# MahdiGhafoorian/NLML_HPE

Measured on AMD Instinct MI355X. Metric: faces_per_sec, higher is better.
Workload: dtype f16x2s

## Files before the change

nlml_hpe_amd/csrc/encoder_heads_f16x2_tailws_dev.h:

```cpp
#pragma once
#include <hip/hip_runtime.h>

#include "../../include/nlml_hpe.h"
#include "abi_internal.h"
#include "encoder_heads_f16x2_dev.h"
#include "layout.h"

#if defined(__HIP_DEVICE_COMPILE__) && !defined(__gfx950__)
#error "global_load_lds_dwordx4: gfx950"
#endif

namespace nlml {
namespace hx {

typedef unsigned u4 __attribute__((ext_vector_type(4)));
#define TW_PRIO(p) __builtin_amdgcn_s_setprio(p)
typedef __attribute__((address_space(3))) const char LdsC;
typedef __attribute__((address_space(3))) char LdsW;

struct TwArgs {
  const void* blob;
  const u4* h3;
  float* out;
  float* latent;
  int64_t B, nfb;
};

constexpr int TW_SLOT = 65536;
constexpr int tw_bias_n16(int s) { return kStages[s].jobs * kStages[s].nb * 8; }
constexpr int tw_bias_off(int s) {
  int o = 0;
  for (int t = ST_E3; t < s; ++t) o += tw_bias_n16(t) * 16;
  return o;
}
constexpr uint32_t tw_b_off(int s, uint32_t k16_e0) {
  int c = (int)(sizeof(Header) / 16), m = 0;
  for (int t = 0; t < s; ++t) {
    c += kStages[t].jobs * ((t == ST_E0 ? 0 : kStages[t].k8 * kStages[t].nb * 64 * PIECES) + kStages[t].nb * 8);
    m += kStages[t].jobs * (t == ST_E0 ? kStages[t].nb * 64 * PIECES : 0);
  }
  return c + m * k16_e0 + kStages[s].jobs * ((s == ST_E0 ? 0 : kStages[s].k8 * kStages[s].nb * 64 * PIECES) + (s == ST_E0 ? kStages[s].nb * 64 * PIECES : 0) * k16_e0);
}
constexpr bool tw_b_off_is_layouts() {
  for (int s = 0; s < NUM_STAGES; ++s)
    if (tw_b_off(s, 0u) != layout_b_off(kLayoutHX, s, 0u) || tw_b_off(s, 88u) != layout_b_off(kLayoutHX, s, 88u)) return false;
  return true;
}
static_assert(tw_b_off_is_layouts(), "the written-out bias offsets are layout.h's");
constexpr int TW_O_BIAS = 2 * TW_SLOT;
constexpr int TW_O_LAT = TW_O_BIAS + ((tw_bias_off(NUM_STAGES) + 511) / 512) * 512;
constexpr int TW_LAT_WAVE = 3 * 2 * 256;
constexpr int TW_LDS = TW_O_LAT + 8 * TW_LAT_WAVE;
static_assert(TW_LDS <= 163840, "LDS map");

constexpr int TW_HEAD_UNITS = 9, TW_UNITS = 4 + 3 * TW_HEAD_UNITS;
constexpr uint32_t tw_job_w16(int s) { return layout_job_w16(kLayoutHX, s, 0u); }
__device__ __forceinline__ void tw_unit(const HdrRegs& H, int idx, uint32_t& off, uint32_t& n16) {
  constexpr uint32_t J3 = tw_job_w16(ST_E3), J4 = tw_job_w16(ST_E4), J5 = tw_job_w16(ST_E5);
  constexpr uint32_t K0 = tw_job_w16(ST_H0), K1 = tw_job_w16(ST_H1), K2 = tw_job_w16(ST_H2), K3 = tw_job_w16(ST_H3), K4 = tw_job_w16(ST_H4);
  static_assert(2 * J3 * 16 == TW_SLOT && 2 * J4 * 16 <= TW_SLOT && J5 * 16 <= TW_SLOT && 4 * K0 * 16 <= TW_SLOT && K1 * 16 <= TW_SLOT &&
                    2 * K2 * 16 == TW_SLOT && 2 * K3 * 16 <= TW_SLOT && K4 * 16 <= TW_SLOT,
                "a unit fits a buffer");
  if (idx < 2) { n16 = 2 * J3; off = H.w_off(ST_E3) + idx * 2 * J3; }
  else if (idx == 2) { n16 = 2 * J4; off = H.w_off(ST_E4); }
  else if (idx == 3) { n16 = J5; off = H.w_off(ST_E5); }
  else {
    const int k = idx - 4, g = k / TW_HEAD_UNITS, r = k - TW_HEAD_UNITS * g;
    if (r == 0) { n16 = 4 * K0; off = H.w_off(ST_H0) + 4 * g * K0; }
    else if (r <= 4) { n16 = K1; off = H.w_off(ST_H1) + (4 * g + (r - 1)) * K1; }
    else if (r <= 6) { n16 = 2 * K2; off = H.w_off(ST_H2) + (4 * g + 2 * (r - 5)) * K2; }
    else if (r == 7) { n16 = 2 * K3; off = H.w_off(ST_H3) + 2 * g * K3; }
    else { n16 = K4; off = H.w_off(ST_H4) + g * K4; }
  }
}

template <int K16, int NCH = 2>
__device__ __forceinline__ void tw_job2(f32x16 (&acc)[2], LdsC* w0, LdsC* w1, int wstep, LdsC* b0, LdsC* b1, const h8 (&in)[K16][2]) {
  typedef const __attribute__((address_space(3))) h8 LdsH8;
#pragma unroll
  for (int c = 0; c < NCH; ++c)
#pragma unroll
    for (int q = 0; q < 4; ++q) {
      const f32x4 v = *reinterpret_cast<const __attribute__((address_space(3))) f32x4*>((c ? b1 : b0) + q * 16);
      acc[c][4 * q + 0] = v[0];
      acc[c][4 * q + 1] = v[1];
      acc[c][4 * q + 2] = v[2];
      acc[c][4 * q + 3] = v[3];
    }
  TW_PRIO(2);
#pragma unroll
  for (int ks = 0; ks < K16; ++ks) {
    h8 wf[NCH][2];
#pragma unroll
    for (int c = 0; c < NCH; ++c)
#pragma unroll
      for (int p = 0; p < 2; ++p) wf[c][p] = *reinterpret_cast<LdsH8*>((c ? w1 : w0) + ks * wstep + p * 1024);
#pragma unroll
    for (int t = 0; t < 3; ++t)
#pragma unroll
      for (int c = 0; c < NCH; ++c)
        acc[c] = __builtin_amdgcn_mfma_f32_32x32x16_f16(wf[c][t == 0 ? 1 : 0], in[ks][t == 1 ? 1 : 0], acc[c], 0, 0, 0);
  }
  TW_PRIO(0);
}

template <int K16>
__device__ __forceinline__ void tw_job2p(f32x16 (&acc)[2], LdsC* w0, LdsC* w1, int wstep, LdsC* b0, LdsC* b1, const h8 (&in)[K16][2]) {
  typedef const __attribute__((address_space(3))) h8 LdsH8;
#pragma unroll
  for (int c = 0; c < 2; ++c)
#pragma unroll
    for (int q = 0; q < 4; ++q) {
      const f32x4 v = *reinterpret_cast<const __attribute__((address_space(3))) f32x4*>((c ? b1 : b0) + q * 16);
      acc[c][4 * q + 0] = v[0];
      acc[c][4 * q + 1] = v[1];
      acc[c][4 * q + 2] = v[2];
      acc[c][4 * q + 3] = v[3];
    }
  h8 wf[2][2][2];
#pragma unroll
  for (int c = 0; c < 2; ++c)
#pragma unroll
    for (int p = 0; p < 2; ++p) wf[0][c][p] = *reinterpret_cast<LdsH8*>((c ? w1 : w0) + p * 1024);
  TW_PRIO(2);
  __builtin_amdgcn_sched_barrier(0);
#pragma unroll
  for (int ks = 0; ks < K16; ++ks) {
#pragma unroll
    for (int m = 0; m < 6; ++m) {
      const int t = m >> 1, c = m & 1;
      acc[c] = __builtin_amdgcn_mfma_f32_32x32x16_f16(wf[ks & 1][c][t == 0 ? 1 : 0], in[ks][t == 1 ? 1 : 0], acc[c], 0, 0, 0);
      __builtin_amdgcn_sched_barrier(0);
      if (m < 4 && ks + 1 < K16)
        wf[(ks + 1) & 1][m & 1][m < 2 ? 1 : 0] = *reinterpret_cast<LdsH8*>(((m & 1) ? w1 : w0) + (ks + 1) * wstep + (m < 2 ? 1024 : 0));
      __builtin_amdgcn_sched_barrier(0);
    }
  }
  TW_PRIO(0);
}

__device__ __forceinline__ void tail_ws_body(const TwArgs& a, int64_t block0, char* const lds) {
  const int tid = threadIdx.x, lane = tid & 63, f = lane & 31, h = lane >> 5;
  const int wv = __builtin_amdgcn_readfirstlane(tid >> 6);
  const HdrRegs H = load_hdr(reinterpret_cast<const Header*>(a.blob));
  const h8* const blob8 = reinterpret_cast<const h8*>(a.blob);
  const f32x4* const blob4 = reinterpret_cast<const f32x4*>(a.blob);

  int64_t fbg = block0 + wv;
  const bool wave_live = fbg < a.nfb;
  fbg = wave_live ? fbg : a.nfb - 1;
  const int64_t row = fbg * 32 + f;
  const bool row_live = wave_live && row < a.B;

  LdsW* const ring = (LdsW*)(lds);
  auto issue = [&](int idx, int slot_off) {
    if (idx >= TW_UNITS) return;
    uint32_t off, n16;
    tw_unit(H, idx, off, n16);
    const int npieces = (int)(n16 >> 6);
#pragma unroll
    for (int i = 0; i < TW_SLOT / 8192; ++i) {
      const int pc = wv + 8 * i;
      if (pc < npieces)
        __builtin_amdgcn_global_load_lds((const __attribute__((address_space(1))) void*)(blob8 + off + pc * 64 + lane),
                                         (__attribute__((address_space(3))) void*)(ring + slot_off + pc * 1024), 16, 0, 0);
    }
  };
#ifdef TW_STAMPS
  int tw_u = 0;
#define TWS(i)                                                                                                                \
  do {                                                                                                                        \
    if (a.latent && lane == 0)                                                                                                \
      reinterpret_cast<unsigned long long*>(a.latent)[((size_t)blockIdx.x * 8 + wv) * 96 + (i)] = __builtin_amdgcn_s_memtime(); \
  } while (0)
#define TW_STAMP_MID() TWS(2 + 2 * tw_u)
#define TW_STAMP_END() do { TWS(3 + 2 * tw_u); ++tw_u; } while (0)
#else
#define TWS(i) do { } while (0)
#define TW_STAMP_MID() do { } while (0)
#define TW_STAMP_END() do { } while (0)
#endif
  TWS(0);
  issue(0, 0);

  {
    f32x4* const bl = reinterpret_cast<f32x4*>(lds + TW_O_BIAS);
#pragma unroll
    for (int s = ST_E3; s < NUM_STAGES; ++s) {
      const f32x4* src = blob4 + tw_b_off(s, H.k8_e0);
      for (int i = tid; i < tw_bias_n16(s); i += 512) bl[tw_bias_off(s) / 16 + i] = src[i];
    }
  }
  h8 x3[TrunkFrags::STEPS][2];
  {
    const u4* src = a.h3 + TrunkFrags::unit(fbg, 0, 0, 0) + lane;
#pragma unroll
    for (int ks = 0; ks < TrunkFrags::STEPS; ++ks)
#pragma unroll
      for (int p = 0; p < 2; ++p) x3[ks][p] = __builtin_bit_cast(h8, src[TrunkFrags::frag(0, ks, p)]);
  }
  asm volatile("s_waitcnt vmcnt(0)" ::: "memory");
  __syncthreads();
  TWS(1);

  int cur = 0;
  LdsC* const bias0 = (LdsC*)(lds + TW_O_BIAS) + 64 * h;
  LdsC* const wl0 = (LdsC*)(lds) + lane * 16;
  LdsW* const latw = (LdsW*)(lds + TW_O_LAT) + wv * TW_LAT_WAVE + f * 8;
#ifdef TW_NO_SKEW
  const bool late = false;
#else
  const bool late = wv >= 4;
#endif
#define TW_BEGIN(idx) issue((idx) + 1, cur ^ TW_SLOT); LdsC* const wl = wl0 + cur
#define TW_MID()                                      \
  TW_STAMP_MID();                                     \
  asm volatile("s_waitcnt vmcnt(0)" ::: "memory");    \
  if (late) __syncthreads()
#define TW_END()                                      \
  asm volatile("s_waitcnt vmcnt(0)" ::: "memory");    \
  if (!late) __syncthreads();                         \
  TW_STAMP_END();                                     \
  cur ^= TW_SLOT

  f32x16 acc[2];
  auto emit = [&](auto act, const f32x16& ac, float inv, h8 (&d0)[2], h8 (&d1)[2]) {
    h8 fr[2][2];
    frags_from_acc<decltype(act)::value>(ac, inv, fr);
    d0[0] = fr[0][0]; d0[1] = fr[0][1]; d1[0] = fr[1][0]; d1[1] = fr[1][1];
  };
  constexpr std::integral_constant<int, ACT_RELU> RELU{};
  constexpr std::integral_constant<int, ACT_TANH> TANH{};
  const float inv3 = H.inv_scale[ST_E3], inv4 = H.inv_scale[ST_E4], inv5 = H.inv_scale[ST_E5];
  constexpr int JB3 = (int)(tw_job_w16(ST_E3) * 16), JB4 = (int)(tw_job_w16(ST_E4) * 16);

  h8 x4[8][2];
#pragma unroll
  for (int u = 0; u < 2; ++u) {
    TW_BEGIN(u);
    LdsC* const b = bias0 + tw_bias_off(ST_E3) + (2 * u) * 128;
    tw_job2p<16>(acc, wl, wl + JB3, 2048, b, b + 128, x3);
    TW_MID();
    emit(RELU, acc[0], inv3, x4[4 * u], x4[4 * u + 1]);
    emit(RELU, acc[1], inv3, x4[4 * u + 2], x4[4 * u + 3]);
    TW_END();
  }
  h8 x5[4][2];
  {
    TW_BEGIN(2);
    LdsC* const b = bias0 + tw_bias_off(ST_E4);
    tw_job2<8>(acc, wl, wl + JB4, 2048, b, b + 128, x4);
    TW_MID();
    emit(TANH, acc[0], inv4, x5[0], x5[1]);
    emit(TANH, acc[1], inv4, x5[2], x5[3]);
    TW_END();
  }
  {
    TW_BEGIN(3);
    LdsC* const b = bias0 + tw_bias_off(ST_E5);
    tw_job2<4>(acc, wl, wl + 2048, 4096, b, b + 128, x5);
    TW_MID();
#ifndef TW_STAMPS
    if (a.latent && row_live) {
#pragma unroll
      for (int nb = 0; nb < 2; ++nb)
#pragma unroll
        for (int q = 0; q < 16; ++q) {
          const int rowi = 32 * nb + (q & 3) + 8 * (q >> 2) + 4 * h, g = rowi >> 4, cc = rowi & 15;
          if (g < 3 && cc < 3) a.latent[row * NLML_LATENT + 3 * g + cc] = acc[nb][q] * inv5;
        }
    }
#endif
#pragma unroll
    for (int nb = 0; nb < 2; ++nb) {
      h8 fr[2][2];
      frags_from_acc<ACT_NONE>(acc[nb], inv5, fr);
#pragma unroll
      for (int p = 0; p < 2; ++p)
#pragma unroll
        for (int pc = 0; pc < 2; ++pc)
          if (2 * nb + p < 3 && h == 0) {
            const u4 t = __builtin_bit_cast(u4, fr[p][pc]);
            typedef unsigned u2 __attribute__((ext_vector_type(2)));
            *reinterpret_cast<__attribute__((address_space(3))) u2*>(latw + ((2 * nb + p) * 2 + pc) * 256) = u2{t[0], t[1]};
          }
    }
    TW_END();
  }
#pragma unroll 1
  for (int g = 0; g < 3; ++g) {
    const int u0 = 4 + TW_HEAD_UNITS * g;
    const float i0 = H.inv_scale[ST_H0], i1 = H.inv_scale[ST_H1], i2 = H.inv_scale[ST_H2], i3 = H.inv_scale[ST_H3];
    h8 xa[8][2];
    {
      TW_BEGIN(u0);
      h8 xin[1][2];
#pragma unroll
      for (int pc = 0; pc < 2; ++pc) {
        typedef unsigned u2 __attribute__((ext_vector_type(2)));
        const u2 t = *reinterpret_cast<const __attribute__((address_space(3))) u2*>((LdsC*)latw + (g * 2 + pc) * 256);
        xin[0][pc] = __builtin_bit_cast(h8, u4{h == 0 ? t[0] : 0u, h == 0 ? t[1] : 0u, 0u, 0u});
      }
      LdsC* const b = bias0 + tw_bias_off(ST_H0) + (4 * g) * 128;
      constexpr int JB = (int)(tw_job_w16(ST_H0) * 16);
#pragma unroll
      for (int jj = 0; jj < 2; ++jj) {
        tw_job2<1>(acc, wl + (2 * jj) * JB, wl + (2 * jj + 1) * JB, 2048, b + (2 * jj) * 128, b + (2 * jj + 1) * 128, xin);
        if (jj == 1) { TW_MID(); }
        emit(RELU, acc[0], i0, xa[4 * jj], xa[4 * jj + 1]);
        emit(RELU, acc[1], i0, xa[4 * jj + 2], xa[4 * jj + 3]);
      }
      TW_END();
    }
    h8 xb[16][2];
#pragma unroll
    for (int j = 0; j < 4; ++j) {
      TW_BEGIN(u0 + 1 + j);
      LdsC* const b = bias0 + tw_bias_off(ST_H1) + (4 * g + j) * 256;
      tw_job2p<8>(acc, wl, wl + 2048, 4096, b, b + 128, xa);
      TW_MID();
      emit(RELU, acc[0], i1, xb[4 * j], xb[4 * j + 1]);
      emit(RELU, acc[1], i1, xb[4 * j + 2], xb[4 * j + 3]);
      TW_END();
    }
    h8 xc[8][2];
#pragma unroll
    for (int u = 0; u < 2; ++u) {
      TW_BEGIN(u0 + 5 + u);
      constexpr int JB = (int)(tw_job_w16(ST_H2) * 16);
      LdsC* const b = bias0 + tw_bias_off(ST_H2) + (4 * g + 2 * u) * 128;
      tw_job2p<16>(acc, wl, wl + JB, 2048, b, b + 128, xb);
      TW_MID();
      emit(RELU, acc[0], i2, xc[4 * u], xc[4 * u + 1]);
      emit(RELU, acc[1], i2, xc[4 * u + 2], xc[4 * u + 3]);
      TW_END();
    }
    h8 xd[4][2];
    {
      TW_BEGIN(u0 + 7);
      LdsC* const b = bias0 + tw_bias_off(ST_H3) + (2 * g) * 128;
      tw_job2p<8>(acc, wl, wl + (int)(tw_job_w16(ST_H3) * 16), 2048, b, b + 128, xc);
      TW_MID();
      emit(RELU, acc[0], i3, xd[0], xd[1]);
      emit(RELU, acc[1], i3, xd[2], xd[3]);
      TW_END();
    }
    {
      TW_BEGIN(u0 + 8);
      LdsC* const b = bias0 + tw_bias_off(ST_H4) + g * 128;
      tw_job2<4, 1>(acc, wl, wl, 2048, b, b, xd);
      TW_MID();
      if (h == 0 && row_live) a.out[row * 3 + g] = acc[0][0] * H.inv_scale[ST_H4];
      TW_END();
    }
  }
#undef TW_BEGIN
#undef TW_MID
#undef TW_END
}

}
}
```

Before: 81.14 million.

## Merge small tail weight units into shared LDS buffers to cut barriers

Packs small consecutive weight units (E4+E5+H0, and H3+H4+next H0) into single double-buffered LDS slots, so the tail goes from 31 units to 24. This removes several waitcnt/__syncthreads seams and prefetch handoffs between tiny jobs. A constexpr checker verifies that the units cover the tail weights in order and fit a slot. The cost is larger per-unit loads with less prefetch lead for the following job, plus more complex control flow.

```diff
diff --git a/nlml_hpe_amd/csrc/encoder_heads_f16x2_tailws_dev.h b/nlml_hpe_amd/csrc/encoder_heads_f16x2_tailws_dev.h
--- a/nlml_hpe_amd/csrc/encoder_heads_f16x2_tailws_dev.h
+++ b/nlml_hpe_amd/csrc/encoder_heads_f16x2_tailws_dev.h
@@ -53,26 +53,70 @@
 constexpr int TW_LDS = TW_O_LAT + 8 * TW_LAT_WAVE;
 static_assert(TW_LDS <= 163840, "LDS map");
 
-constexpr int TW_HEAD_UNITS = 9, TW_UNITS = 4 + 3 * TW_HEAD_UNITS;
+struct TwSeg { int stage, job0, jobs; };
+struct TwUnit { TwSeg seg[3]; };
+#ifdef TW_NO_MERGE
+constexpr int TW_ENC_UNITS = 4, TW_HEAD_UNITS = 9;
+#else
+constexpr int TW_ENC_UNITS = 3, TW_HEAD_UNITS = 7;
+#endif
+constexpr int TW_KINDS = TW_ENC_UNITS + TW_HEAD_UNITS, TW_UNITS = TW_ENC_UNITS + 3 * TW_HEAD_UNITS;
+#ifdef TW_NO_MERGE
+constexpr int TW_K_E4 = 2, TW_K_E5 = 3, TW_K_H0 = 4, TW_K_H1 = 5, TW_K_H2 = 9, TW_K_H3 = 11, TW_K_H4 = 12;
+#else
+constexpr int TW_K_E4 = 2, TW_K_E5 = 2, TW_K_H1 = 3, TW_K_H2 = 7, TW_K_H3 = 9, TW_K_H4 = 9;
+#endif
+constexpr TwUnit tw_unit(int k, int g) {
+  if (k < 2) return {{{ST_E3, 2 * k, 2}, {}, {}}};
+#ifdef TW_NO_MERGE
+  if (k == TW_K_E4) return {{{ST_E4, 0, 2}, {}, {}}};
+  if (k == TW_K_E5) return {{{ST_E5, 0, 1}, {}, {}}};
+  if (k == TW_K_H0) return {{{ST_H0, 4 * g, 4}, {}, {}}};
+  if (k < TW_K_H2) return {{{ST_H1, 4 * g + (k - TW_K_H1), 1}, {}, {}}};
+  if (k < TW_K_H3) return {{{ST_H2, 4 * g + 2 * (k - TW_K_H2), 2}, {}, {}}};
+  if (k == TW_K_H3) return {{{ST_H3, 2 * g, 2}, {}, {}}};
+  return {{{ST_H4, g, 1}, {}, {}}};
+#else
+  if (k == TW_K_E4) return {{{ST_E4, 0, 2}, {ST_E5, 0, 1}, {ST_H0, 0, 4}}};
+  if (k < TW_K_H2) return {{{ST_H1, 4 * g + (k - TW_K_H1), 1}, {}, {}}};
+  if (k < TW_K_H3) return {{{ST_H2, 4 * g + 2 * (k - TW_K_H2), 2}, {}, {}}};
+  return {{{ST_H3, 2 * g, 2}, {ST_H4, g, 1}, {ST_H0, 4 * (g + 1), g < 2 ? 4 : 0}}};
+#endif
+}
 constexpr uint32_t tw_job_w16(int s) { return layout_job_w16(kLayoutHX, s, 0u); }
-__device__ __forceinline__ void tw_unit(const HdrRegs& H, int idx, uint32_t& off, uint32_t& n16) {
-  constexpr uint32_t J3 = tw_job_w16(ST_E3), J4 = tw_job_w16(ST_E4), J5 = tw_job_w16(ST_E5);
-  constexpr uint32_t K0 = tw_job_w16(ST_H0), K1 = tw_job_w16(ST_H1), K2 = tw_job_w16(ST_H2), K3 = tw_job_w16(ST_H3), K4 = tw_job_w16(ST_H4);
-  static_assert(2 * J3 * 16 == TW_SLOT && 2 * J4 * 16 <= TW_SLOT && J5 * 16 <= TW_SLOT && 4 * K0 * 16 <= TW_SLOT && K1 * 16 <= TW_SLOT &&
-                    2 * K2 * 16 == TW_SLOT && 2 * K3 * 16 <= TW_SLOT && K4 * 16 <= TW_SLOT,
-                "a unit fits a buffer");
-  if (idx < 2) { n16 = 2 * J3; off = H.w_off(ST_E3) + idx * 2 * J3; }
-  else if (idx == 2) { n16 = 2 * J4; off = H.w_off(ST_E4); }
-  else if (idx == 3) { n16 = J5; off = H.w_off(ST_E5); }
-  else {
-    const int k = idx - 4, g = k / TW_HEAD_UNITS, r = k - TW_HEAD_UNITS * g;
-    if (r == 0) { n16 = 4 * K0; off = H.w_off(ST_H0) + 4 * g * K0; }
-    else if (r <= 4) { n16 = K1; off = H.w_off(ST_H1) + (4 * g + (r - 1)) * K1; }
-    else if (r <= 6) { n16 = 2 * K2; off = H.w_off(ST_H2) + (4 * g + 2 * (r - 5)) * K2; }
-    else if (r == 7) { n16 = 2 * K3; off = H.w_off(ST_H3) + 2 * g * K3; }
-    else { n16 = K4; off = H.w_off(ST_H4) + g * K4; }
-  }
-}
+constexpr int tw_seg_pieces(const TwSeg& s) { return s.jobs * (int)(tw_job_w16(s.stage) >> 6); }
+constexpr bool tw_units_are_the_tail() {
+  int next[NUM_STAGES] = {};
+  for (int idx = 0; idx < TW_UNITS; ++idx) {
+    const int k = idx < TW_ENC_UNITS ? idx : TW_ENC_UNITS + (idx - TW_ENC_UNITS) % TW_HEAD_UNITS;
+    const int g = idx < TW_ENC_UNITS ? 0 : (idx - TW_ENC_UNITS) / TW_HEAD_UNITS;
+    const TwUnit U = tw_unit(k, g);
+    int pieces = 0;
+    for (int j = 0; j < 3; ++j) {
+      const TwSeg s = U.seg[j];
+      if (s.jobs == 0) continue;
+      if (s.stage < ST_E3 || s.stage >= NUM_STAGES || s.job0 != next[s.stage] || tw_seg_pieces(s) % 8 != 0) return false;
+      if ((tw_job_w16(s.stage) & 63u) != 0) return false;
+      if (s.stage > ST_E3) {
+        const int p = s.stage - 1;
+        const int need = s.stage <= ST_H0 ? kStages[p].jobs : ((s.job0 + s.jobs - 1) / (kStages[s.stage].jobs / 3) + 1) * (kStages[p].jobs / 3);
+        if (next[p] < need) return false;
+      }
+      next[s.stage] += s.jobs;
+      pieces += tw_seg_pieces(s);
+    }
+    if (pieces == 0 || pieces * 1024 > TW_SLOT) return false;
+  }
+  for (int s = ST_E3; s < NUM_STAGES; ++s)
+    if (next[s] != kStages[s].jobs) return false;
+  return true;
+}
+static_assert(tw_units_are_the_tail(), "the units cover the tail's weights exactly once, in the order of use, each within a buffer");
+#ifndef TW_NO_MERGE
+static_assert(TW_UNITS == 24 && (2 * tw_job_w16(ST_E4) + tw_job_w16(ST_E5) + 4 * tw_job_w16(ST_H0)) * 16 == 56 * 1024 &&
+                  (2 * tw_job_w16(ST_H3) + tw_job_w16(ST_H4) + 4 * tw_job_w16(ST_H0)) * 16 == 48 * 1024,
+              "E4 + E5 + H0 is 56 KB, H3 + H4 + H0 is 48 KB");
+#endif
 
 template <int K16, int NCH = 2>
 __device__ __forceinline__ void tw_job2(f32x16 (&acc)[2], LdsC* w0, LdsC* w1, int wstep, LdsC* b0, LdsC* b1, const h8 (&in)[K16][2]) {
@@ -153,18 +197,30 @@
   const bool row_live = wave_live && row < a.B;
 
   LdsW* const ring = (LdsW*)(lds);
-  auto issue = [&](int idx, int slot_off) {
-    if (idx >= TW_UNITS) return;
-    uint32_t off, n16;
-    tw_unit(H, idx, off, n16);
-    const int npieces = (int)(n16 >> 6);
-#pragma unroll
-    for (int i = 0; i < TW_SLOT / 8192; ++i) {
-      const int pc = wv + 8 * i;
-      if (pc < npieces)
-        __builtin_amdgcn_global_load_lds((const __attribute__((address_space(1))) void*)(blob8 + off + pc * 64 + lane),
-                                         (__attribute__((address_space(3))) void*)(ring + slot_off + pc * 1024), 16, 0, 0);
-    }
+  auto issue = [&](int k, int g, int slot_off) {
+    const TwUnit U = tw_unit(k, g);
+    int first = 0;
+    unsigned lane16 = lane * 16;
+    asm volatile("" : "+v"(lane16));
+#pragma unroll
+    for (int j = 0; j < 3; ++j) {
+      const int np = tw_seg_pieces(U.seg[j]);
+      const uint32_t off = H.w_off(U.seg[j].stage) + U.seg[j].job0 * tw_job_w16(U.seg[j].stage);
+#pragma unroll
+      for (int i = 0; i < TW_SLOT / 8192; ++i) {
+        const int pc = wv + 8 * i;
+        if (8 * i >= first && 8 * i < first + np) {
+          const char* const piece = reinterpret_cast<const char*>(a.blob) + (size_t)(off + (pc - first) * 64) * 16;
+          __builtin_amdgcn_global_load_lds((const __attribute__((address_space(1))) void*)(piece + lane16),
+                                           (__attribute__((address_space(3))) void*)(ring + slot_off + pc * 1024), 16, 0, 0);
+        }
+      }
+      first += np;
+    }
+  };
+  auto issue_next = [&](int k, int g, int slot_off) {
+    if (k + 1 < TW_KINDS) issue(k + 1, g, slot_off);
+    else if (g < 2) issue(TW_ENC_UNITS, g + 1, slot_off);
   };
 #ifdef TW_STAMPS
   int tw_u = 0;
@@ -181,7 +237,7 @@
 #define TW_STAMP_END() do { } while (0)
 #endif
   TWS(0);
-  issue(0, 0);
+  issue(0, 0, 0);
 
   {
     f32x4* const bl = reinterpret_cast<f32x4*>(lds + TW_O_BIAS);
@@ -212,7 +268,8 @@
 #else
   const bool late = wv >= 4;
 #endif
-#define TW_BEGIN(idx) issue((idx) + 1, cur ^ TW_SLOT); LdsC* const wl = wl0 + cur
+  LdsC* wl;
+#define TW_BEGIN(k, g) issue_next(k, g, cur ^ TW_SLOT); wl = wl0 + cur
 #define TW_MID()                                      \
   TW_STAMP_MID();                                     \
   asm volatile("s_waitcnt vmcnt(0)" ::: "memory");    \
@@ -222,6 +279,13 @@
   if (!late) __syncthreads();                         \
   TW_STAMP_END();                                     \
   cur ^= TW_SLOT
+#ifdef TW_NO_MERGE
+#define TW_SEAM_MID() TW_MID()
+#define TW_SEAM_END(k, g, bytes) TW_END(); TW_BEGIN(k, g)
+#else
+#define TW_SEAM_MID() do { } while (0)
+#define TW_SEAM_END(k, g, bytes) wl += (bytes)
+#endif
 
   f32x16 acc[2];
   auto emit = [&](auto act, const f32x16& ac, float inv, h8 (&d0)[2], h8 (&d1)[2]) {
@@ -232,12 +296,32 @@
   constexpr std::integral_constant<int, ACT_RELU> RELU{};
   constexpr std::integral_constant<int, ACT_TANH> TANH{};
   const float inv3 = H.inv_scale[ST_E3], inv4 = H.inv_scale[ST_E4], inv5 = H.inv_scale[ST_E5];
-  constexpr int JB3 = (int)(tw_job_w16(ST_E3) * 16), JB4 = (int)(tw_job_w16(ST_E4) * 16);
+  constexpr int JB3 = (int)(tw_job_w16(ST_E3) * 16), JB4 = (int)(tw_job_w16(ST_E4) * 16), JB5 = (int)(tw_job_w16(ST_E5) * 16);
+  constexpr int JBH0 = (int)(tw_job_w16(ST_H0) * 16), JBH3 = (int)(tw_job_w16(ST_H3) * 16), JBH4 = (int)(tw_job_w16(ST_H4) * 16);
+
+  auto h0_front = [&](int gg, LdsC* w, h8 (&xa)[8][2]) {
+    h8 xin[1][2];
+#pragma unroll
+    for (int pc = 0; pc < 2; ++pc) {
+      typedef unsigned u2 __attribute__((ext_vector_type(2)));
+      const u2 t = *reinterpret_cast<const __attribute__((address_space(3))) u2*>((LdsC*)latw + (gg * 2 + pc) * 256);
+      xin[0][pc] = __builtin_bit_cast(h8, u4{h == 0 ? t[0] : 0u, h == 0 ? t[1] : 0u, 0u, 0u});
+    }
+    LdsC* const b = bias0 + tw_bias_off(ST_H0) + (4 * gg) * 128;
+    tw_job2<1>(acc, w, w + JBH0, 2048, b, b + 128, xin);
+    emit(RELU, acc[0], H.inv_scale[ST_H0], xa[0], xa[1]);
+    emit(RELU, acc[1], H.inv_scale[ST_H0], xa[2], xa[3]);
+    tw_job2<1>(acc, w + 2 * JBH0, w + 3 * JBH0, 2048, b + 2 * 128, b + 3 * 128, xin);
+  };
+  auto h0_back = [&](h8 (&xa)[8][2]) {
+    emit(RELU, acc[0], H.inv_scale[ST_H0], xa[4], xa[5]);
+    emit(RELU, acc[1], H.inv_scale[ST_H0], xa[6], xa[7]);
+  };
 
   h8 x4[8][2];
 #pragma unroll
   for (int u = 0; u < 2; ++u) {
-    TW_BEGIN(u);
+    TW_BEGIN(u, 0);
     LdsC* const b = bias0 + tw_bias_off(ST_E3) + (2 * u) * 128;
     tw_job2p<16>(acc, wl, wl + JB3, 2048, b, b + 128, x3);
     TW_MID();
@@ -247,19 +331,19 @@
   }
   h8 x5[4][2];
   {
-    TW_BEGIN(2);
+    TW_BEGIN(TW_K_E4, 0);
     LdsC* const b = bias0 + tw_bias_off(ST_E4);
     tw_job2<8>(acc, wl, wl + JB4, 2048, b, b + 128, x4);
-    TW_MID();
+    TW_SEAM_MID();
     emit(TANH, acc[0], inv4, x5[0], x5[1]);
     emit(TANH, acc[1], inv4, x5[2], x5[3]);
-    TW_END();
-  }
+    TW_SEAM_END(TW_K_E5, 0, 2 * JB4);
+  }
+  h8 xa[8][2];
   {
-    TW_BEGIN(3);
     LdsC* const b = bias0 + tw_bias_off(ST_E5);
     tw_job2<4>(acc, wl, wl + 2048, 4096, b, b + 128, x5);
-    TW_MID();
+    TW_SEAM_MID();
 #ifndef TW_STAMPS
     if (a.latent && row_live) {
 #pragma unroll
@@ -285,37 +369,32 @@
             *reinterpret_cast<__attribute__((address_space(3))) u2*>(latw + ((2 * nb + p) * 2 + pc) * 256) = u2{t[0], t[1]};
           }
     }
+#ifdef TW_NO_MERGE
     TW_END();
+#else
+    wl += JB5;
+    h0_front(0, wl, xa);
+    TW_MID();
+    h0_back(xa);
+    TW_END();
+#endif
   }
 #pragma unroll 1
   for (int g = 0; g < 3; ++g) {
-    const int u0 = 4 + TW_HEAD_UNITS * g;
-    const float i0 = H.inv_scale[ST_H0], i1 = H.inv_scale[ST_H1], i2 = H.inv_scale[ST_H2], i3 = H.inv_scale[ST_H3];
-    h8 xa[8][2];
+    const float i1 = H.inv_scale[ST_H1], i2 = H.inv_scale[ST_H2], i3 = H.inv_scale[ST_H3];
+#ifdef TW_NO_MERGE
     {
-      TW_BEGIN(u0);
-      h8 xin[1][2];
-#pragma unroll
-      for (int pc = 0; pc < 2; ++pc) {
-        typedef unsigned u2 __attribute__((ext_vector_type(2)));
-        const u2 t = *reinterpret_cast<const __attribute__((address_space(3))) u2*>((LdsC*)latw + (g * 2 + pc) * 256);
-        xin[0][pc] = __builtin_bit_cast(h8, u4{h == 0 ? t[0] : 0u, h == 0 ? t[1] : 0u, 0u, 0u});
-      }
-      LdsC* const b = bias0 + tw_bias_off(ST_H0) + (4 * g) * 128;
-      constexpr int JB = (int)(tw_job_w16(ST_H0) * 16);
-#pragma unroll
-      for (int jj = 0; jj < 2; ++jj) {
-        tw_job2<1>(acc, wl + (2 * jj) * JB, wl + (2 * jj + 1) * JB, 2048, b + (2 * jj) * 128, b + (2 * jj + 1) * 128, xin);
-        if (jj == 1) { TW_MID(); }
-        emit(RELU, acc[0], i0, xa[4 * jj], xa[4 * jj + 1]);
-        emit(RELU, acc[1], i0, xa[4 * jj + 2], xa[4 * jj + 3]);
-      }
+      TW_BEGIN(TW_K_H0, g);
+      h0_front(g, wl, xa);
+      TW_MID();
+      h0_back(xa);
       TW_END();
     }
+#endif
     h8 xb[16][2];
 #pragma unroll
     for (int j = 0; j < 4; ++j) {
-      TW_BEGIN(u0 + 1 + j);
+      TW_BEGIN(TW_K_H1 + j, g);
       LdsC* const b = bias0 + tw_bias_off(ST_H1) + (4 * g + j) * 256;
       tw_job2p<8>(acc, wl, wl + 2048, 4096, b, b + 128, xa);
       TW_MID();
@@ -326,7 +405,7 @@
     h8 xc[8][2];
 #pragma unroll
     for (int u = 0; u < 2; ++u) {
-      TW_BEGIN(u0 + 5 + u);
+      TW_BEGIN(TW_K_H2 + u, g);
       constexpr int JB = (int)(tw_job_w16(ST_H2) * 16);
       LdsC* const b = bias0 + tw_bias_off(ST_H2) + (4 * g + 2 * u) * 128;
       tw_job2p<16>(acc, wl, wl + JB, 2048, b, b + 128, xb);
@@ -337,27 +416,41 @@
     }
     h8 xd[4][2];
     {
-      TW_BEGIN(u0 + 7);
+      TW_BEGIN(TW_K_H3, g);
       LdsC* const b = bias0 + tw_bias_off(ST_H3) + (2 * g) * 128;
-      tw_job2p<8>(acc, wl, wl + (int)(tw_job_w16(ST_H3) * 16), 2048, b, b + 128, xc);
-      TW_MID();
+      tw_job2p<8>(acc, wl, wl + JBH3, 2048, b, b + 128, xc);
+      TW_SEAM_MID();
       emit(RELU, acc[0], i3, xd[0], xd[1]);
       emit(RELU, acc[1], i3, xd[2], xd[3]);
-      TW_END();
+      TW_SEAM_END(TW_K_H4, g, 2 * JBH3);
     }
     {
-      TW_BEGIN(u0 + 8);
       LdsC* const b = bias0 + tw_bias_off(ST_H4) + g * 128;
       tw_job2<4, 1>(acc, wl, wl, 2048, b, b, xd);
+#ifdef TW_NO_MERGE
       TW_MID();
       if (h == 0 && row_live) a.out[row * 3 + g] = acc[0][0] * H.inv_scale[ST_H4];
       TW_END();
-    }
-  }
+#else
+      if (h == 0 && row_live) a.out[row * 3 + g] = acc[0][0] * H.inv_scale[ST_H4];
+      if (g == 2) break;
+      h0_front(g + 1, wl + JBH4, xa);
+      TW_MID();
+      h0_back(xa);
+      TW_END();
+#endif
+    }
+  }
+#ifndef TW_NO_MERGE
+  TW_MID();
+  TW_END();
+#endif
 #undef TW_BEGIN
 #undef TW_MID
 #undef TW_END
-}
-
-}
-}
+#undef TW_SEAM_MID
+#undef TW_SEAM_END
+}
+
+}
+}
```

After: 81.51 million, median of 6. About the same (+0.5%).
